# OpenDrift/opendrift

Measured on AMD Instinct MI355X. Metric: particle-steps/sec (RK4, 3D interp), higher is better.
Workload: dtype f64; 1 GPU; C3: OceanDrift 3D, synthetic ROMS-shaped z-level grid 1024x1024x12 (u,v,w,K), RK4 + vertical_mixing(60 s) + vertical_advection; particles_per_gpu=10000000, particles_total=10000000, stage_math=fast, spin_up_steps=200, block_every=0, inputs=resident in HBM, parallelism=particle-sharded x1, field block broadcast once per time level

## Files before the change

include/odrift.h:

```cpp
#ifndef ODRIFT_H
#define ODRIFT_H
#include <stdint.h>

#ifdef __cplusplus
extern "C" {
#endif

typedef struct odr_ctx odr_ctx;
typedef struct odr_particles odr_particles;

typedef enum {
  ODR_OK = 0,
  ODR_ERR_INVALID = -1,
  ODR_ERR_HIP = -2,
  ODR_ERR_CAPACITY = -3,
  ODR_ERR_STATE = -4
} odr_status;

enum {
  ODR_VAR_X_SEA_WATER_VELOCITY = 0,
  ODR_VAR_Y_SEA_WATER_VELOCITY = 1,
  ODR_VAR_X_WIND = 2,
  ODR_VAR_Y_WIND = 3,
  ODR_VAR_UPWARD_SEA_WATER_VELOCITY = 4,
// ... 251 lines not shown
                         double dt_seconds, int rng_mode, const double *u1, const double *u2, const double *diameter_noise,
                         const double *depth_noise, uint64_t step);
int odr_radio_terminal_velocity(odr_ctx *ctx, odr_particles *p, int diameter_slot, int density_slot);
int odr_radio_resuspend(odr_ctx *ctx, odr_particles *p, odr_radio *radio, int specie_slot, int diameter_slot, int rng_mode,
                        const double *diameter_noise, const double *depth_noise, uint64_t step);
int odr_particles_count_status(odr_ctx *ctx, odr_particles *p, int32_t status_code, int64_t *n);
int odr_particles_remap_status(odr_ctx *ctx, odr_particles *p, int32_t from_code, int32_t to_code);
int odr_deactivate(odr_ctx *ctx, odr_particles *p, const uint8_t *mask_host, int32_t status_code);
int odr_deactivate_outside(odr_ctx *ctx, odr_particles *p, double west, double east, double south, double north,
                           int32_t status_code);
int odr_compact(odr_ctx *ctx, odr_particles *p, int64_t *n_active);
int odr_scan_status(odr_ctx *ctx, odr_particles *p, int64_t *n_kept, uint64_t *status_flags);
int odr_scan_status_begin(odr_ctx *ctx, odr_particles *p);
int odr_scan_status_end(odr_ctx *ctx, odr_particles *p, int64_t *n_kept, uint64_t *status_flags);
int odr_ctx_guard_next_vmix(odr_ctx *ctx, int on);
int odr_compact_apply(odr_ctx *ctx, odr_particles *p, int64_t *n_active);
int odr_sort_particles(odr_ctx *ctx, odr_particles *p, int32_t source_id);
int odr_sort_particles_ex(odr_ctx *ctx, odr_particles *p, int32_t source_id, int keep_environment);
int odr_particles_tile_stats(odr_ctx *ctx, odr_particles *p, uint64_t *out4);
int odr_particles_step_layout_stats(odr_ctx *ctx, odr_particles *p, uint64_t *out2);
int odr_particles_step_onlevel_stats(odr_ctx *ctx, odr_particles *p, uint64_t *out1);
int odr_particles_vmix_layout_stats(odr_ctx *ctx, odr_particles *p, uint64_t *out3);
int odr_particles_vmix_kplane_stats(odr_ctx *ctx, odr_particles *p, uint64_t *out2);
int odr_reduce_scalars(odr_ctx *ctx, odr_particles *p, double wind_drift_depth, double *out16);
int odr_ctx_set_step_reduce(odr_ctx *ctx, int on, double wind_drift_depth, int relative_wind);
int odr_reduce_local(odr_ctx *ctx, odr_particles *p, double wind_drift_depth, int relative_wind, double *out16);
int odr_reduce_install(odr_ctx *ctx, odr_particles *p, const double *in16);
int odr_reduce_unpin(odr_ctx *ctx);

int odr_ctx_set_position_class(odr_ctx *ctx, int f32);
int odr_source_set_coordinate_dtype(odr_ctx *ctx, int32_t source_id, int x_is_float32, int y_is_float32);

#define ODR_COMM_ID_BYTES 256
int odr_device_count(int32_t *n);
int odr_comm_unique_id(uint8_t *id );
int odr_comm_init(odr_ctx *ctx, const uint8_t *id, int32_t rank, int32_t nranks);
int odr_comm_info(int32_t *rank, int32_t *nranks, uint64_t *id_hash, int32_t *rccl_version, uint64_t *collectives);
int odr_comm_destroy(void);
int odr_allreduce_scalars(odr_ctx *ctx, double *values, int32_t n, int32_t op);
int odr_comm_allgather_begin(odr_ctx *ctx, const double *row, int32_t n, int32_t from_scan);
int odr_comm_allgather_end(odr_ctx *ctx, double *rows );
int odr_comm_broadcast_bytes(odr_ctx *ctx, void *buf, int64_t nbytes, int32_t root);
int odr_comm_barrier(odr_ctx *ctx);
int odr_block_broadcast(odr_ctx *ctx, int32_t source_id, int32_t slot, double t_epoch, int nvars, const int32_t *var_ids,
                        const void *const *data, const int32_t *var_nz, int ny, int nx, const double *xy8, int32_t root);

// ... 91 lines not shown
```

opendrift_amd/_abi.py:

```python
import ctypes as C
import os

HERE = os.path.dirname(os.path.abspath(__file__))
LIB_PATH = os.environ.get('ODR_LIB') or os.path.join(HERE, 'libodrift_hip.so')

NVAR = 26
VARIABLES = {
    'x_sea_water_velocity': 0, 'y_sea_water_velocity': 1, 'x_wind': 2, 'y_wind': 3,
    'upward_sea_water_velocity': 4, 'ocean_vertical_diffusivity': 5,
    'sea_surface_wave_stokes_drift_x_velocity': 6, 'sea_surface_wave_stokes_drift_y_velocity': 7,
    'land_binary_mask': 8, 'sea_floor_depth_below_sea_level': 9, 'sea_surface_height': 10,
    'horizontal_diffusivity': 11, 'sea_surface_wave_significant_height': 12,
    'sea_surface_wave_period_at_variance_spectral_density_maximum': 13,
    'ocean_mixed_layer_thickness': 14,
    'sea_water_temperature': 15, 'sea_water_salinity': 16,
    'sea_ice_area_fraction': 17, 'sea_ice_x_velocity': 18, 'sea_ice_y_velocity': 19,
    'sea_surface_swell_wave_to_direction': 20,
    'sea_surface_swell_wave_peak_period_from_variance_spectral_density': 21,
    'sea_surface_swell_wave_significant_height': 22, 'sea_surface_wind_wave_to_direction': 23,
    'sea_surface_wind_wave_mean_period': 24, 'sea_surface_wind_wave_significant_height': 25,
}
VARIABLE_NAMES = {v: k for k, v in VARIABLES.items()}
PROJ_LATLONG, PROJ_STERE_EQUIT_SPHERE, PROJ_STERE_POLAR = 0, 1, 2
PROJ_MERC, PROJ_LCC = 4, 5
# ... 151 lines not shown
    'odr_device_count': [_P(C.c_int32)],
    'odr_comm_unique_id': [_P(C.c_uint8)],
    'odr_comm_init': [_vp, _P(C.c_uint8), C.c_int32, C.c_int32],
    'odr_comm_info': [_P(C.c_int32), _P(C.c_int32), _P(C.c_uint64), _P(C.c_int32), _P(C.c_uint64)],
    'odr_comm_destroy': [],
    'odr_allreduce_scalars': [_vp, _dp, C.c_int32, C.c_int32],
    'odr_comm_allgather_begin': [_vp, _dp, C.c_int32, C.c_int32],
    'odr_comm_allgather_end': [_vp, _dp],
    'odr_comm_broadcast_bytes': [_vp, _vp, C.c_int64, C.c_int32],
    'odr_comm_barrier': [_vp],
    'odr_block_broadcast': [_vp, C.c_int32, C.c_int32, C.c_double, C.c_int, _ip, _P(_vp), _ip, C.c_int, C.c_int, _dp, C.c_int32],
    'odr_scan_status': [_vp, _vp, _i64p, _P(C.c_uint64)],
    'odr_scan_status_begin': [_vp, _vp],
    'odr_scan_status_end': [_vp, _vp, _i64p, _P(C.c_uint64)],
    'odr_ctx_guard_next_vmix': [_vp, C.c_int],
    'odr_compact_apply': [_vp, _vp, _i64p],
    'odr_sort_particles': [_vp, _vp, C.c_int32],
    'odr_sort_particles_ex': [_vp, _vp, C.c_int32, C.c_int],
    'odr_particles_tile_stats': [_vp, _vp, _P(C.c_uint64)],
    'odr_particles_step_layout_stats': [_vp, _vp, _P(C.c_uint64)],
    'odr_particles_step_onlevel_stats': [_vp, _vp, _P(C.c_uint64)],
    'odr_particles_vmix_layout_stats': [_vp, _vp, _P(C.c_uint64)],
    'odr_particles_vmix_kplane_stats': [_vp, _vp, _P(C.c_uint64)],
    'odr_reduce_scalars': [_vp, _vp, C.c_double, _dp],
    'odr_ctx_set_step_reduce': [_vp, C.c_int, C.c_double, C.c_int],
    'odr_reduce_local': [_vp, _vp, C.c_double, C.c_int, _dp],
    'odr_reduce_install': [_vp, _vp, _dp],
    'odr_reduce_unpin': [_vp],
    'odr_timer_begin': [_vp],
    'odr_timer_end': [_vp, _fp],
    'odr_sgrid_create': [_vp, C.c_int32, C.c_int32, C.c_int32, _dp, _dp, C.c_double, _dp, _dp, C.c_int32, _P(_vp)],
    'odr_sgrid_destroy': [_vp, _vp],
    'odr_sgrid_download_zrho': [_vp, _vp, _dp],
    'odr_sgrid_zslice': [_vp, _vp, _vp, C.c_int, C.c_int, C.c_int32, _dp, C.c_int32, _P(_vp), _dp],
    'odr_history_create': [_vp, C.c_int64, C.c_int32, C.c_int32, _ip, _P(_vp)],
    'odr_history_destroy': [_vp, _vp],
    'odr_history_set_id_base': [_vp, _vp, C.c_int64],
    'odr_history_record': [_vp, _vp, _vp, C.c_int32, C.c_int, C.c_int],
    'odr_history_flush': [_vp, _vp, C.c_int32, C.c_int32],
    'odr_history_wait': [_vp, _vp],
    'odr_history_host_ptr': [_vp, _vp, C.c_int32, _P(_fp), _P(C.c_int32)],
    'odr_history_reset': [_vp, _vp],
    'odr_history_minmax': [_vp, _vp, C.c_int32, _dp, _dp],
    'odr_density_map': [_vp, C.c_int64, C.c_int32] + [_vp] * 5 + [C.c_int32, C.c_int32, _dp, C.c_int32, _dp, _dp, _dp, _dp],
    'odr_density_last_kernel_ms': [_vp, _fp],
    'odr_density_map_proj': [_vp, C.c_int64, C.c_int32] + [_vp] * 5 + [C.c_int32, _P(ProjDesc), C.c_int32, _dp, C.c_int32, _dp, C.c_int64, _dp, _dp, _dp],
# ... 77 lines not shown
```

opendrift_amd/csrc/odr_host.h:

```cpp
#pragma once
#include <hip/hip_runtime.h>

#include <algorithm>
#include <cmath>
#include <cstdarg>
#include <cstdio>
#include <cstdlib>
#include <cstring>
#include <initializer_list>
#include <string>
#include <vector>

#include "../../include/odrift.h"
#include "odr_kernels.hip.h"

using namespace odr;

#include <chrono>
struct SlowSpan {
  const char *what;
  std::chrono::steady_clock::time_point t0;
  static double limit() { static const double v = getenv("ODR_SLOW_CALLS") ? atof(getenv("ODR_SLOW_CALLS")) : 0.0; return v; }
  explicit SlowSpan(const char *w) : what(w) { if (limit() > 0) t0 = std::chrono::steady_clock::now(); }
  ~SlowSpan() {
// ... 107 lines not shown
  long long aux_snap_cap[9];
  double *dead64[3];
  int *deadi32[2];
  unsigned *bcount;
  unsigned *wcount;
  unsigned long long wcount_epoch;
  long long wcount_n;
  void *scratch;
  size_t scratch_bytes;
  unsigned long long epoch;
  unsigned long long status_epoch, scan_epoch;
  long long scan_kept;
  float env_cval[NVAR];
  long long env_cn[NVAR];
  bool env_cok[NVAR];
  bool external;
  unsigned *wg_tab, *wg_list;
  unsigned long long *wg_total, *wg_stats;
  long long wg_cap, wg_grid, wg_n, wg_list_cap;
  unsigned long long wg_launches;
  unsigned long long step_launches[3];
  unsigned long long vmix_launches[3];
  unsigned long long vmix_kplane[2];
  double *z_keep;
  long long z_keep_n;
  bool z_truncated;
  int wg_sid;
  bool wg_valid;
  unsigned wg_src_gen;
};

static inline unsigned nblk(long long n) { return (unsigned)((n + BLOCK - 1) / BLOCK); }

static inline PView view(const odr_particles *p) {
  PView v;
  v.n = p->n;
  v.lon = p->d64[0]; v.lat = p->d64[1]; v.z = p->d64[2]; v.plon = p->d64[3]; v.plat = p->d64[4];
  v.slon = p->d64[5]; v.slat = p->d64[6];
  v.id = p->i32[0]; v.status = p->i32[1]; v.moving = p->i32[2];
  v.wdf = p->f32[0]; v.cdf = p->f32[1]; v.tv = p->f32[2]; v.age = p->f32[3];
  for (int k = 0; k < NVAR; ++k) v.env[k] = p->env[k];
  for (int k = 0; k < 9; ++k) v.aux[k] = p->aux[k];
  v.ice = p->ice_kind; v.pad = 0;
  v.rank = p->rank_on && p->rank ? p->rank : nullptr;
  return v;
}
// ... 179 lines not shown
```

opendrift_amd/csrc/odr_kernels.hip.h:

```cpp
#pragma once
#include <hip/hip_runtime.h>
#include <rocrand/rocrand_kernel.h>
#include "odr_field.hip.h"

namespace odr {

#ifndef ODR_BLOCK
#define ODR_BLOCK 256
#endif
constexpr int BLOCK = ODR_BLOCK;
#ifndef ODR_POLAR_WAVES
#define ODR_POLAR_WAVES 3
#endif
#ifndef ODR_POLAR_STEP_WAVES
#define ODR_POLAR_STEP_WAVES 2
#endif
#define ODR_STEP_WAVES(PROJ) ((PROJ) == PROJ_LATLONG ? ODR_LATLONG_WAVES : ((PROJ) == PROJ_EXT ? 1 : ODR_POLAR_STEP_WAVES))
#ifndef ODR_LATLONG_WAVES
#define ODR_LATLONG_WAVES 1
#endif
#define ODR_WAVES(PROJ) ((PROJ) == PROJ_LATLONG ? ODR_LATLONG_WAVES : ((PROJ) == PROJ_EXT ? 1 : ODR_POLAR_WAVES))

__device__ __forceinline__ long long pid() {
  const unsigned nb = gridDim.x, b = blockIdx.x, per = nb >> 3, rem = nb & 7u, x = b & 7u, j = b >> 3;
// ... 321 lines not shown
__device__ __forceinline__ unsigned mix_word(const uint4 &q, unsigned k) {
  const unsigned lo = ((q.x & 255u) << 16) | ((q.y & 255u) << 8) | (q.z & 255u);
  return k == 0 ? q.x >> 8 : (k == 1 ? q.y >> 8 : (k == 2 ? q.z >> 8 : (k == 3 ? q.w >> 8 : lo)));
}
__device__ __forceinline__ unsigned mix_draw(const MixKey &K, uint4 &q, int it, bool primed = false) {
  const unsigned b = (unsigned)it / 5u, k = (unsigned)it - 5u * b;
  if (k == 0 && !(primed && it == 0)) q = mix_block(K, b);
  return mix_word(q, k);
}
__device__ __forceinline__ double mix_uniform(const MixKey &K, uint4 &q, int it, bool primed = false) {
  return ((double)mix_draw(K, q, it, primed) + 0.5) * 5.9604644775390625e-08;
}
__device__ __forceinline__ double mix_R_of(unsigned x) {
  return (double)((int)(2u * x + 1u) - (1 << 24)) * 5.9604644775390625e-08;
}
constexpr int AUX_KMEMBER = 8;
struct VMixDesc {
  int sid, nzp, geo_slot;
  unsigned kstride;
  const float *kb, *ka;
  double wgt;
  float Kfb, pad2;
  const unsigned long long *guard;
};

struct VMixRT {
  static constexpr bool STATIC = false;
  __host__ __device__ static constexpr int proj_kind(int k) { return k; }
  __host__ __device__ static constexpr int lon_mode(int m) { return m; }
  __host__ __device__ static constexpr int mod360_x(int m) { return m; }
  __host__ __device__ static constexpr int nzp(int n, int ) { return n; }
  __host__ __device__ static constexpr bool uniform_z(bool u) { return u; }
  __host__ __device__ static constexpr int rng_mode(int m) { return m; }
  __host__ __device__ static constexpr int mix_at_surface(int m) { return m; }
  __host__ __device__ static constexpr int sf_action(int a) { return a; }
  __host__ __device__ static constexpr int vadv(int v) { return v; }
  __host__ __device__ static constexpr int ntimes(int n) { return n; }
  __host__ __device__ static constexpr unsigned kstride(unsigned b, int ) { return b; }
  __device__ static void proj_fwd(const DevProj &p, double lon, double lat, double &x, double &y) { proj_fwd_rt(p, lon, lat, x, y); }
};
struct VMixC3 {
  static constexpr bool STATIC = true;
  __host__ __device__ static constexpr int proj_kind(int) { return PROJ_LATLONG; }
  __host__ __device__ static constexpr int lon_mode(int) { return 1; }
  __host__ __device__ static constexpr int mod360_x(int) { return 0; }
  __host__ __device__ static constexpr int nzp(int, int NL) { return NL; }
  __host__ __device__ static constexpr bool uniform_z(bool) { return false; }
  __host__ __device__ static constexpr int rng_mode(int) { return 0; }
  __host__ __device__ static constexpr int mix_at_surface(int) { return 0; }
  __host__ __device__ static constexpr int sf_action(int) { return 1; }
  __host__ __device__ static constexpr int vadv(int) { return 0; }
  __host__ __device__ static constexpr int ntimes(int) { return 10; }
  __host__ __device__ static constexpr unsigned kstride(unsigned, int NQ) { return 16u * (unsigned)NQ; }
  __device__ static void proj_fwd(const DevProj &, double lon, double lat, double &x, double &y) { x = lon; y = lat; }
};

struct VMixC3Rec : VMixC3 {
  __host__ __device__ static constexpr unsigned kstride(unsigned b, int ) { return b; }
};

template <int NQ, bool TL, class VM, class HOOK>
__device__ __forceinline__ void vmix_col_fill(const DevSource &s, const VMixDesc &D, double lon, double lat, double *Kp,
                                              int tid, HOOK &&hook) {
  const double Kfb = (double)D.Kfb;
  double x, y;
  const int lon_mode = VM::lon_mode(s.lon_mode);
  if (lon_mode == 1) lon = np_mod(lon + 180.0, 360.0) - 180.0;
  else if (lon_mode == 2) lon = np_mod(lon, 360.0);
  VM::proj_fwd(s.proj, lon, lat, x, y);
  const bool cov = x >= s.xmin && x <= s.xmax && y >= s.ymin && y <= s.ymax;
  if (VM::mod360_x(s.mod360_x)) x = np_mod(x, 360.0);
  const DevBlock &bb = s.slot[D.geo_slot];
  const double xi = __dmul_rn(div_cr(x - bb.x0, bb.xspan, bb.ixspan), (double)(bb.nx - 1));
  const double yi = __dmul_rn(div_cr(y - bb.y0, bb.yspan, bb.iyspan), (double)(bb.ny - 1));
  const int ny = bb.ny, nx = bb.nx;
  const Axis ay = axis_fp(yi, ny), ax = axis_fp(xi, nx);
  const double ty = ay.t, tx = ax.t, wy0 = 1 - ty, wx0 = 1 - tx, wgt = D.wgt;
  const unsigned recb = VM::kstride(D.kstride, NQ);
  const unsigned r0 = __umul24((unsigned)ay.i0, (unsigned)nx), r1 = __umul24((unsigned)ay.i1, (unsigned)nx);
  const unsigned o00 = cov ? __umul24(r0 + (unsigned)ax.i0, recb) : 0u, o01 = cov ? __umul24(r0 + (unsigned)ax.i1, recb) : 0u;
  const unsigned o10 = cov ? __umul24(r1 + (unsigned)ax.i0, recb) : 0u, o11 = cov ? __umul24(r1 + (unsigned)ax.i1, recb) : 0u;
  const float *kb = D.kb, *ka = TL ? D.ka : D.kb;
  const double w00 = wy0 * wx0, w01 = wy0 * tx, w10 = ty * wx0, w11 = ty * tx;
#pragma unroll
  for (int q = 0; q < NQ; ++q) {
    if (VM::STATIC && q > 0) __builtin_amdgcn_sched_barrier(0);
    const F4 b00 = ld_off<F4>(kb, o00 + 16u * q), b01 = ld_off<F4>(kb, o01 + 16u * q);
    const F4 b10 = ld_off<F4>(kb, o10 + 16u * q), b11 = ld_off<F4>(kb, o11 + 16u * q);
    F4 a00, a01, a10, a11;
    if (TL) {
      a00 = ld_off<F4>(ka, o00 + 16u * q); a01 = ld_off<F4>(ka, o01 + 16u * q);
      a10 = ld_off<F4>(ka, o10 + 16u * q); a11 = ld_off<F4>(ka, o11 + 16u * q);
    }
    if (VM::STATIC && q > 0) __builtin_amdgcn_sched_barrier(0);
    if (q == 0) hook();
    double v[4];
    v[0] = (double)bilw(b00.x, b01.x, b10.x, b11.x, w00, w01, w10, w11);
    v[1] = (double)bilw(b00.y, b01.y, b10.y, b11.y, w00, w01, w10, w11);
    v[2] = (double)bilw(b00.z, b01.z, b10.z, b11.z, w00, w01, w10, w11);
    v[3] = (double)bilw(b00.w, b01.w, b10.w, b11.w, w00, w01, w10, w11);
    if (TL) {
      double w[4];
      w[0] = (double)bilw(a00.x, a01.x, a10.x, a11.x, w00, w01, w10, w11);
      w[1] = (double)bilw(a00.y, a01.y, a10.y, a11.y, w00, w01, w10, w11);
      w[2] = (double)bilw(a00.z, a01.z, a10.z, a11.z, w00, w01, w10, w11);
      w[3] = (double)bilw(a00.w, a01.w, a10.w, a11.w, w00, w01, w10, w11);
#pragma unroll
      for (int j = 0; j < 4; ++j) v[j] = __dadd_rn(__dmul_rn(v[j], 1 - wgt), __dmul_rn(w[j], wgt));
// ... 2 lines not shown
    for (int j = 0; j < 4; ++j) Kp[(4 * q + j) * BLOCK + tid] = (cov && isfinite(v[j])) ? v[j] : Kfb;
  }
}

struct VMixArgs {
  double dt, dt_mix_cfg;
  int mix_at_surface, rng_mode, sfl, pad;
  const double *huni;
  unsigned long long seed, step;
};
struct MixRng { MixKey key; uint4 q; bool primed; };
template <class VM = VMixRT>
__device__ __forceinline__ MixRng mix_rng_begin(const VMixArgs &A, int id) {
  MixRng R;
  R.key = mix_key(A.seed, A.step, id);
  R.q = make_uint4(0u, 0u, 0u, 0u);
  R.primed = false;
  if (VM::rng_mode(A.rng_mode) == 0) {
    R.q = mix_block(R.key, 0u);
    R.primed = true;
  }
  return R;
}
template <int NQ, class VM = VMixRT>
__device__ __forceinline__ double vmix_col_walk(const DevSource &s, int nzp, const double *Kp, const double *gsh, int tid,
                                                const VMixArgs &A, long long i, long long n, int id, double z, int &moving,
                                                float Zmin, float tv, int &sf_flags, const MixRng *pre) {
  constexpr int NL = 4 * NQ;
  static_assert(!VM::STATIC || NL >= 3, "a static configuration has the three-level window inside the profile");
  const double dt = A.dt;
  const int mix_at_surface = VM::mix_at_surface(A.mix_at_surface), rng_mode = VM::rng_mode(A.rng_mode), sfl = A.sfl;
  double zm[NL - 1];
#pragma unroll
  for (int k = 0; k < NL - 1; ++k) zm[k] = k < nzp - 1 ? s.zmid[k] : __builtin_inf();
  const bool uniform_z = VM::uniform_z(s.vg_uniform != 0);
  const double gd0 = s.vg_d[0], gi0 = s.vg_id[0], gd1 = s.vg_d[1], gi1 = s.vg_id[1], gd2 = s.vg_d[2], gi2 = s.vg_id[2];
  const double sgn = dt > 0 ? 1.0 : (dt < 0 ? -1.0 : 0.0);
  const double dt_mix = A.dt_mix_cfg * sgn;
  const int ntimes = VM::ntimes(abs((int)(dt / dt_mix)));
  const double r = 1.0 / 3, ir = 1.0 / r;
  double wstep = __dmul_rn(__dmul_rn((double)tv, dt_mix), (double)moving);
  const MixKey st = mix_key(A.seed, A.step, id);
  uint4 u4 = make_uint4(0u, 0u, 0u, 0u);
  bool primed = false;
  if (pre) { u4 = pre->q; primed = pre->primed; }
  auto level_terms = [&](auto edges, int zl, double &dk_dt, double &sg) {
    constexpr int E = decltype(edges)::value;
    const double Kz = Kp[zl * BLOCK + tid];
    double gK;
    if ((E & 1) && zl == 0) gK = div_cr(Kp[BLOCK + tid] - Kz, gd0, gi0);
    else if ((E & 2) && zl == nzp - 1) gK = div_cr(Kz - Kp[(nzp - 2) * BLOCK + tid], gd1, gi1);
    else if (uniform_z) gK = div_cr(Kp[(zl + 1) * BLOCK + tid] - Kp[(zl - 1) * BLOCK + tid], gd2, gi2);
    else
      gK = __dadd_rn(__dadd_rn(__dmul_rn(gsh[zl], Kp[(zl - 1) * BLOCK + tid]), __dmul_rn(gsh[NL + zl], Kz)),
                     __dmul_rn(gsh[2 * NL + zl], Kp[(zl + 1) * BLOCK + tid]));
    double dK = -gK;
    if (fabs(dK) < 1e-10) dK = 0;
    dk_dt = __dmul_rn(dK, dt_mix);
    sg = sqrt(div_cr(__dmul_rn(__dmul_rn(Kz, fabs(dt_mix)), 2.0), r, ir));
  };
  using AnyLevel = std::integral_constant<int, 3>;
  int lv0;
  {
    const double d0 = -z;
    int zs = 0;
#pragma unroll
    for (int k = 0; k < NL - 1; ++k) zs += ((k & 1) ? d0 >= zm[k] : d0 > zm[k]) ? 1 : 0;
    lv0 = zs < 1 ? 1 : (zs > nzp - 2 ? nzp - 2 : zs);
    if (nzp < 3) lv0 = 1;
  }
  double c_dk[3], c_sg[3];
#pragma unroll
  for (int q = 0; q < 3; ++q) {
    const int zl = lv0 - 1 + q;
    c_dk[q] = 0; c_sg[q] = 0;
    if constexpr (VM::STATIC) {
      if (q == 0) level_terms(std::integral_constant<int, 1>(), zl, c_dk[q], c_sg[q]);
      else if (q == 1) level_terms(std::integral_constant<int, 0>(), zl, c_dk[q], c_sg[q]);
      else level_terms(std::integral_constant<int, 2>(), zl, c_dk[q], c_sg[q]);
    } else if (zl >= 0 && zl < nzp) level_terms(AnyLevel(), zl, c_dk[q], c_sg[q]);
  }
  double wb[4];
#pragma unroll
  for (int j = 0; j < 4; ++j) {
    const int k = lv0 - 2 + j;
    double b = k < 0 ? -1.0 : __builtin_inf();
    if (k >= 0 && k < nzp - 1) {
      b = gsh[3 * NL + k];
      if ((k & 1) && b > 0) b = __longlong_as_double(__double_as_longlong(b) - 1);
    }
    wb[j] = b;
  }
  for (int it0 = 0; it0 < ntimes; it0 += 5) {
  if (rng_mode == 0 && !(primed && it0 == 0)) u4 = mix_block(st, (unsigned)it0 / 5u);
#pragma unroll
  for (int k5 = 0; k5 < 5; ++k5) {
    const int it = it0 + k5;
    if (it >= ntimes) break;
    const bool surface = z == 0;
    const double d = -z;
    int q = (d > wb[1] ? 1 : 0) + (d > wb[2] ? 1 : 0);
    int zi = lv0 - 1 + q;
    if (!(d > wb[0]) || d > wb[3]) {
      zi = 0;
#pragma unroll
      for (int k = 0; k < NL - 1; ++k) zi += ((k & 1) ? d >= zm[k] : d > zm[k]) ? 1 : 0;
      q = zi - lv0 + 1;
    }
    double dKdt = q == 0 ? c_dk[0] : (q == 1 ? c_dk[1] : c_dk[2]);
    double sig = q == 0 ? c_sg[0] : (q == 1 ? c_sg[1] : c_sg[2]);
    if (q < 0 || q > 2) level_terms(AnyLevel(), zi, dKdt, sig);
    double R;
    if (rng_mode == 1) R = __dsub_rn(__dmul_rn(2.0, A.huni[(size_t)it * n + i]), 1.0);
    else R = mix_R_of(mix_word(u4, (unsigned)k5));
    z = __dsub_rn(z, __dmul_rn((double)moving, __dsub_rn(dKdt, __dmul_rn(R, sig))));
    if (z >= 0) z = -z;
    if (z < (double)Zmin && moving == 1) z = __dsub_rn((double)__fmul_rn(2.f, Zmin), z);
    z = __dadd_rn(z, wstep);
    if (!mix_at_surface && surface) z = 0.0;
    if (z > 0) z = 0.0;
    if (z < (double)Zmin) {
      const int act = VM::sf_action(sfl & 255);
      if (act == 3) sf_flags |= 2;
      else if (act) {
        z = (double)Zmin;
        if (act == 2) { sf_flags |= 1; moving = 0; wstep = 0.0; }
        else if (act == 4) { sf_flags |= 4; moving = 0; wstep = 0.0; }
        else if (act == 5 && (sf_flags & 8)) { sf_flags |= 4; moving = 0; wstep = 0.0; }
      }
    }
  }
  }
  return z;
}
// ... 1047 lines not shown
  if (vadv >= 0 && (vadv ? z <= 0 : z < 0)) {
    double zz = __dadd_rn(z, __dmul_rn(__dmul_rn((double)moving, (double)p.env[VAR_W][i]), dt));
    z = zz < 0 ? zz : 0.0;
  }
  if (OIL) {
    p.tv[i] = (float)oil.W;
    p.aux[OIL_DIAMETER][i] = oil.d;
  }
  p.z[i] = z;
}

#ifndef ODR_VMIX_WAVES
#define ODR_VMIX_WAVES 6
#endif
struct VMixState { double slon, slat, z0; int moving, id; float dep, ssh, tv; };
__device__ __forceinline__ VMixState vmix_load_state(const PView &p, long long i) {
  VMixState S;
  S.slon = p.slon[i]; S.slat = p.slat[i]; S.z0 = p.z[i];
  S.moving = p.moving[i]; S.id = p.id[i];
  S.dep = p.env[VAR_DEPTH][i]; S.ssh = p.env[VAR_SSH][i]; S.tv = p.tv[i];
  return S;
}
template <int NQ, bool TL, class VM>
__device__ __forceinline__ void vmix_col_particle(const DevSource &s, const PView &p, const VMixDesc &D, const VMixArgs &A,
                                                  int vadv, long long i, double *Kp, const double *gsh, int tid, const VMixState &S) {
  const int nzp = VM::nzp(D.nzp, 4 * NQ), sfl = A.sfl;
  const double dt = A.dt;
  const double slon = S.slon, slat = S.slat, z0 = S.z0;
  int moving = S.moving;
  const float dep0 = S.dep, ssh0 = S.ssh, tv0 = S.tv;
  const int id0 = S.id;
  MixRng R0;
  R0.key = mix_key(A.seed, A.step, id0); R0.q = make_uint4(0u, 0u, 0u, 0u); R0.primed = false;
  vmix_col_fill<NQ, TL, VM>(s, D, slon, slat, Kp, tid, [&]() { R0 = mix_rng_begin<VM>(A, id0); });
  int sf_flags = VM::sf_action(sfl & 255) == 5 ? sf_species_flag(p, sfl, i) : 0;
  const float Zmin = __fmul_rn(-1.f, __fadd_rn(dep0, ssh0));
  double z = vmix_col_walk<NQ, VM>(s, nzp, Kp, gsh, tid, A, i, p.n, id0, z0, moving, Zmin, tv0, sf_flags, &R0);
  if (sf_flags & 1) {
    if (p.status[i] == 0) p.status[i] = sfl >> 8;
    p.moving[i] = 0;
  }
  if (sf_flags & 4) p.moving[i] = 0;
  if (sf_flags & 2) { p.lon[i] = p.plon[i]; p.lat[i] = p.plat[i]; }
  vadv = VM::vadv(vadv);
  if (vadv >= 0 && (vadv ? z <= 0 : z < 0)) {
    const float w0 = p.env[VAR_W][i];
    double zz = __dadd_rn(z, __dmul_rn(__dmul_rn((double)moving, (double)w0), dt));
    z = zz < 0 ? zz : 0.0;
  }
  p.z[i] = z;
}
template <int NQ, bool TL, class VM = VMixRT>
__global__ __launch_bounds__(BLOCK, ODR_VMIX_WAVES) void k_vmix_col(const DevWorld *__restrict__ W, PView p, VMixDesc D,
                                                    double dt, double dt_mix_cfg, int mix_at_surface,
                                                    int rng_mode, const double *__restrict__ huni,
                                                    unsigned long long seed, unsigned long long step,
                                                    int vadv, int sfl) {
  constexpr int NL = 4 * NQ;
  extern __shared__ __attribute__((aligned(16))) char smem[];
  const int tid = threadIdx.x;
  const DevSource &s = W->src[D.sid];
  const int nzp = VM::nzp(D.nzp, NL);
  double *Kp = (double *)smem;
  double *gsh = Kp + (size_t)NL * BLOCK;
  if (D.guard && *D.guard == 0ull) return;
  const long long i = pid();
  const bool valid = i < p.n;
  const VMixState S = vmix_load_state(p, valid ? i : 0);
  if (tid < nzp) {
    gsh[tid] = s.vg_a[tid]; gsh[NL + tid] = s.vg_b[tid]; gsh[2 * NL + tid] = s.vg_c[tid];
    gsh[3 * NL + tid] = s.zmid[tid];
  }
  __syncthreads();
  if (!valid) return;
  VMixArgs A;
  A.dt = dt; A.dt_mix_cfg = dt_mix_cfg; A.mix_at_surface = mix_at_surface; A.rng_mode = rng_mode; A.sfl = sfl; A.pad = 0;
  A.huni = huni; A.seed = seed; A.step = step;
  vmix_col_particle<NQ, TL, VM>(s, p, D, A, vadv, i, Kp, gsh, tid, S);
}

#ifndef ODR_VWIN_WAVES
#define ODR_VWIN_WAVES 5
#endif
template <bool TL>
__device__ __forceinline__ double vmix_layer(float b00, float b01, float b10, float b11, float a00, float a01, float a10, float a11,
                                             double w00, double w01, double w10, double w11, double wgt, bool cov, double Kfb) {
  double v = (double)bilw(b00, b01, b10, b11, w00, w01, w10, w11);
  if (TL) {
    const double w = (double)bilw(a00, a01, a10, a11, w00, w01, w10, w11);
    v = __dadd_rn(__dmul_rn(v, 1 - wgt), __dmul_rn(w, wgt));
  }
  return (cov && isfinite(v)) ? v : Kfb;
}
struct VMixGrad { double gd0, gi0, gd1, gi1, gd2, gi2, dt_mix; bool uniform_z; };
__device__ __forceinline__ void vmix_terms(const VMixGrad &G, const double *gsh, int nzp, int zl, double Kl, double Kz, double Kh,
                                           double &dk_dt, double &sg) {
  const double r = 1.0 / 3, ir = 1.0 / r;
  double gK;
  if (zl == 0) gK = div_cr(Kh - Kz, G.gd0, G.gi0);
  else if (zl == nzp - 1) gK = div_cr(Kz - Kl, G.gd1, G.gi1);
  else if (G.uniform_z) gK = div_cr(Kh - Kl, G.gd2, G.gi2);
// ... 1448 lines not shown
```

opendrift_amd/csrc/odr_mix.hip:

```cpp
#define ODR_TU_MIX 1
#include "odr_host.h"

template <class VM>
static bool vmix_layout_matches(const DevSource &s, const VMixDesc &D, int nq, double dt, double dt_mix, int mix_at_surface,
                                int rng_mode, int sfl, int vadv) {
  const bool uz = s.vg_uniform != 0;
  const int ntimes = abs((int)(dt / (dt_mix * (dt > 0 ? 1.0 : (dt < 0 ? -1.0 : 0.0)))));
  return VM::proj_kind(s.proj.kind) == s.proj.kind && VM::lon_mode(s.lon_mode) == s.lon_mode &&
         VM::mod360_x(s.mod360_x) == s.mod360_x && VM::nzp(D.nzp, 4 * nq) == D.nzp && VM::uniform_z(uz) == uz &&
         VM::rng_mode(rng_mode) == rng_mode && VM::mix_at_surface(mix_at_surface) == mix_at_surface &&
         VM::sf_action(sfl & 255) == (sfl & 255) && VM::vadv(vadv) == vadv && VM::ntimes(ntimes) == ntimes &&
         VM::kstride(D.kstride, nq) == D.kstride;
}

int odr_vmix(odr_ctx *c, odr_particles *p, double t, double dt, double dt_mix, int mix_at_surface, int rng_mode,
             const double *huni, uint64_t step) {
  const bool guarded = c->guard_next_vmix != 0;
  c->guard_next_vmix = 0;
  const bool oil = c->oil_owner == p;
  const bool f32prof = p->profiles_f32;
  const int cut = c->vmix_levels;
  VMixDesc D;
  bool kplanes = !getenv("ODR_NO_KPLANE");
  const bool fast = !oil && !f32prof && cut <= 0 && !getenv("ODR_NO_FAST_PATH") && build_vmix_desc(c, t, D, kplanes);
// ... 34 lines not shown
  unsigned long long st = (unsigned long long)step;
  if (vadv >= 0 && !p->env[VAR_W]) return fail(ODR_ERR_STATE, "upward_sea_water_velocity has not been sampled");
  struct F32ProfileClass {
    odr_ctx *c;
    bool on;
    ~F32ProfileClass() { if (on) { c->hw.f32pos &= ~2; c->dirty = true; } }
  } f32bit{c, false};
  if (f32prof) { c->hw.f32pos |= 2; c->dirty = true; f32bit.on = true; if ((rc = flush_world(c))) return rc; }
  if (cut > 0) {
    REQUIRE(cut >= 2 && cut <= 255, "odr_vmix_set_profile_levels: 2 .. 255 levels");
    if (cut < nzp) nzp = cut;
  }
  const int sfl_cut = c->seafloor | ((cut > 0 ? nzp : 0) << 16);
  if (fast) {
    if (guarded) { D.guard = c->counter + 4; c->guarded_vmix = p; c->guarded_vadv = vadv; }
    const int nq = (nzp + 3) / 4;
    const bool tl = D.ka != nullptr;
    const char *wenv = getenv("ODR_VMIX_WINDOW");
    const bool win = nzp >= 3 && nzp <= BLOCK && (wenv ? atoi(wenv) != 0 : nzp > 12);
    const bool spec = !win && (nq == 2 || nq == 3) &&
                      vmix_layout_matches<VMixC3Rec>(c->hw.src[D.sid], D, nq, dt, dt_mix, mix_at_surface, rng_mode, c->seafloor, vadv) &&
                      !getenv("ODR_NO_VMIX_SPEC");
    const bool specp = spec && vmix_layout_matches<VMixC3>(c->hw.src[D.sid], D, nq, dt, dt_mix, mix_at_surface, rng_mode, c->seafloor, vadv);
    p->vmix_launches[win ? 2 : spec ? 1 : 0]++;
    p->vmix_kplane[kplanes ? 0 : 1]++;
#define VMIX_COL(NQ, VM)                                                                                          \
  do {                                                                                                            \
    size_t l2 = sizeof(double) * ((size_t)(4 * NQ) * BLOCK + 4 * (size_t)(4 * NQ));                               \
    if (tl) hipLaunchKernelGGL((k_vmix_col<NQ, true, VM>), g, b, l2, c->stream, c->dw, v, D, dt, dt_mix,          \
                               mix_at_surface, rng_mode, du, c->seed, st, vadv, c->seafloor);                                  \
    else hipLaunchKernelGGL((k_vmix_col<NQ, false, VM>), g, b, l2, c->stream, c->dw, v, D, dt, dt_mix,            \
                            mix_at_surface, rng_mode, du, c->seed, st, vadv, c->seafloor);                                     \
  } while (0)
    if (win) {
      const size_t lw = (sizeof(double) + sizeof(unsigned)) * 4 * BLOCK + sizeof(double) * 4 * (size_t)nzp;
      if (tl) hipLaunchKernelGGL((k_vmix_win<true>), g, b, lw, c->stream, c->dw, v, D, dt, dt_mix, mix_at_surface, rng_mode, du,
                                 c->seed, st, vadv, c->seafloor);
      else hipLaunchKernelGGL((k_vmix_win<false>), g, b, lw, c->stream, c->dw, v, D, dt, dt_mix, mix_at_surface, rng_mode, du,
                              c->seed, st, vadv, c->seafloor);
    }
    else if (specp && nq == 2) VMIX_COL(2, VMixC3);
    else if (specp) VMIX_COL(3, VMixC3);
    else if (spec && nq == 2) VMIX_COL(2, VMixC3Rec);
    else if (spec) VMIX_COL(3, VMixC3Rec);
    else if (nq <= 1) VMIX_COL(1, VMixRT);
    else if (nq == 2) VMIX_COL(2, VMixRT);
    else if (nq == 3) VMIX_COL(3, VMixRT);
    else if (nq == 4) VMIX_COL(4, VMixRT);
    else if (nq <= 6) VMIX_COL(6, VMixRT);
    else if (nq <= 8) VMIX_COL(8, VMixRT);
    else if (nq <= 12) VMIX_COL(12, VMixRT);
    else VMIX_COL(16, VMixRT);
#undef VMIX_COL
  } else if (oil) {
    if (nzp <= 16) hipLaunchKernelGGL((k_vmix<16, true>), g, b, lds, c->stream, c->dw, v, t, dt, dt_mix, mix_at_surface, rng_mode, du, c->seed, st, vadv, sfl_cut, c->oil);
    else if (nzp <= 32) hipLaunchKernelGGL((k_vmix<32, true>), g, b, lds, c->stream, c->dw, v, t, dt, dt_mix, mix_at_surface, rng_mode, du, c->seed, st, vadv, sfl_cut, c->oil);
    else hipLaunchKernelGGL((k_vmix<1, true>), g, b, lds, c->stream, c->dw, v, t, dt, dt_mix, mix_at_surface, rng_mode, du, c->seed, st, vadv, sfl_cut, c->oil);
  } else if (nzp <= 16) hipLaunchKernelGGL(k_vmix<16>, g, b, lds, c->stream, c->dw, v, t, dt, dt_mix, mix_at_surface, rng_mode, du, c->seed, st, vadv, sfl_cut);
  else if (nzp <= 32) hipLaunchKernelGGL(k_vmix<32>, g, b, lds, c->stream, c->dw, v, t, dt, dt_mix, mix_at_surface, rng_mode, du, c->seed, st, vadv, sfl_cut);
  else hipLaunchKernelGGL(k_vmix<1>, g, b, lds, c->stream, c->dw, v, t, dt, dt_mix, mix_at_surface, rng_mode, du, c->seed, st, vadv, sfl_cut);
  if (!fast) p->vmix_launches[2]++;
  HIPCHK(hipGetLastError());
  return 0;
}

int odr_particles_vmix_layout_stats(odr_ctx *c, odr_particles *p, uint64_t *out3) {
  REQUIRE(c && p && out3, "NULL argument");
  for (int k = 0; k < 3; ++k) out3[k] = p->vmix_launches[k];
  return 0;
}

int odr_particles_vmix_kplane_stats(odr_ctx *c, odr_particles *p, uint64_t *out2) {
  REQUIRE(c && p && out2, "NULL argument");
  out2[0] = p->vmix_kplane[0]; out2[1] = p->vmix_kplane[1];
  return 0;
}

int odr_vmix_set_profile_levels(odr_ctx *c, int32_t n) {
  REQUIRE(n == 0 || (n >= 2 && n <= 255), "bad level count %d", n);
  c->vmix_levels = n;
  return 0;
}

int odr_vmix_wind_profile(odr_ctx *c, odr_particles *p, int model, double background_diffusivity, double dt,
                          double dt_mix, int mix_at_surface, int rng_mode, const double *huni, uint64_t step) {
  c->guard_next_vmix = 0;
  p->status_epoch++;
  p->epoch++;
  REQUIRE(model == ODR_DIFFUSIVITY_LARGE1994 || model == ODR_DIFFUSIVITY_SUNDBY1983, "Unknown diffusivity model: %d", model);
  REQUIRE(dt_mix > 0 && dt != 0, "bad time steps");
  if (!p->env[VAR_DEPTH]) return fail(ODR_ERR_STATE, "sea_floor_depth_below_sea_level has not been sampled");
  int rc;
  if ((rc = seafloor_species_slot_ok(c, p))) return rc;
  for (int v : {VAR_SSH, VAR_XWIND, VAR_YWIND, VAR_MLD})
    if ((rc = ensure_env(c, p, v))) return rc;
  if ((rc = flush_world(c))) return rc;
  if (p->n == 0) return 0;
// ... 162 lines not shown
```

opendrift_amd/csrc/odrift.hip:

```cpp
#define ODR_TU_MISC 1
#include "odr_host.h"
#include "odr_mesh.h"

static thread_local std::string g_err;
int odr_i_fail(int code, const char *fmt, ...) {
  char buf[512];
  va_list ap;
  va_start(ap, fmt);
  vsnprintf(buf, sizeof buf, fmt, ap);
  va_end(ap);
  g_err = buf;
  return code;
}

const char *odr_last_error(void) { return g_err.c_str(); }
#define ODR_STR2(x) #x
#define ODR_STR(x) ODR_STR2(x)
const char *odr_version(void) { return "odrift-hip 0.2 (gfx950; mixing stream Philox4x32-" ODR_STR(ODR_MIX_ROUNDS) ")"; }

int odr_ctx_create(int device, uint64_t seed, odr_ctx **out) {
  REQUIRE(out, "out is NULL");
  HIPCHK(hipSetDevice(device));
  odr_ctx *c = new odr_ctx();
  c->device = device;
// ... 79 lines not shown
  return 0;
}
int odr_timer_end(odr_ctx *c, float *ms) {
  HIPCHK(hipEventRecord(c->ev1, c->stream));
  HIPCHK(hipEventSynchronize(c->ev1));
  HIPCHK(hipEventElapsedTime(ms, c->ev0, c->ev1));
  return 0;
}

int odr_particles_create(odr_ctx *c, int64_t capacity, odr_particles **out) {
  REQUIRE(capacity > 0 && out, "capacity must be positive");
  HIPCHK(hipSetDevice(c->device));
  odr_particles *p = new odr_particles();
  memset(p, 0, sizeof(*p));
  p->cap = capacity;
  p->dead_cap = capacity;
  p->scan_kept = -1;
  for (int k = 0; k < 7; ++k) HIPCHK(hipMalloc((void **)&p->d64[k], sizeof(double) * (size_t)capacity));
  for (int k = 0; k < 3; ++k) HIPCHK(hipMalloc((void **)&p->i32[k], sizeof(int) * (size_t)capacity));
  for (int k = 0; k < 4; ++k) HIPCHK(hipMalloc((void **)&p->f32[k], sizeof(float) * (size_t)capacity));
  HIPCHK(hipMalloc((void **)&p->bcount, sizeof(unsigned) * (size_t)(nblk(capacity) + 1)));
  HIPCHK(hipMalloc((void **)&p->wcount, sizeof(unsigned) * (size_t)(nblk(capacity) + 1) * (BLOCK / 64)));
  p->wcount_epoch = ~0ull;
  *out = p;
  return 0;
}

int odr_particles_destroy(odr_ctx *c, odr_particles *p) {
  if (c->red_owner == p) c->red_owner = nullptr;
  if (c->noise_owner == p) c->noise_owner = nullptr;
  if (c->guarded_vmix == p) c->guarded_vmix = nullptr;
  if (!p) return 0;
  (void)hipStreamSynchronize(c->stream);
  auto fr = [](void *q) { if (q) (void)hipFree(q); };
  for (int k = 0; k < 7; ++k) { fr(p->d64[k]); fr(p->alt64[k]); }
  for (int k = 0; k < 3; ++k) { fr(p->i32[k]); fr(p->alti32[k]); fr(p->dead64[k]); }
  for (int k = 0; k < 4; ++k) { fr(p->f32[k]); fr(p->altf32[k]); }
  for (int k = 0; k < 2; ++k) fr(p->deadi32[k]);
  for (int k = 0; k < NVAR; ++k) { fr(p->env[k]); fr(p->altenv[k]); }
  for (int k = 0; k < 9; ++k) { fr(p->aux[k]); fr(p->altaux[k]); fr(p->aux_snap[k]); }
  fr(p->bcount);
  fr(p->wcount);
  fr(p->scratch);
  fr(p->rank); fr(p->rank_words); fr(p->rank_before); fr(p->rank_bsum);
  fr(p->wg_tab); fr(p->wg_total); fr(p->wg_list); fr(p->z_keep);
  delete p;
  return 0;
}

template <class T>
static int put(odr_ctx *c, T *dst, const T *src, long long n, T dflt) {
  if (src) {
    H2D(dst, src, sizeof(T) * (size_t)n);
  } else {
    std::vector<T> tmp((size_t)n, dflt);
    H2D(dst, tmp.data(), sizeof(T) * (size_t)n);
    HIPCHK(hipStreamSynchronize(c->stream));
  }
  return 0;
}

int odr_particles_append(odr_ctx *c, odr_particles *p, int64_t n, const double *lon, const double *lat,
                         const double *z, const int32_t *id, const int32_t *moving, const float *wdf,
                         const float *cdf, const float *tv) {
  p->status_epoch++;
// ... 2410 lines not shown
```

opendrift_amd/device.py:

```python
import ctypes as C
import os

import numpy as np

from . import _abi
from ._abi import VARIABLES, check

_dp, _fp, _ip = C.POINTER(C.c_double), C.POINTER(C.c_float), C.POINTER(C.c_int32)


def _vid(v, aliases=None):
    if isinstance(v, (int, np.integer)):
        return v
    if v in VARIABLES:
        return VARIABLES[v]
    if aliases and v in aliases:
        return aliases[v]
    raise KeyError(v)


def _d(a, n=None):
    if a is None:
        return None, None
    a = np.ascontiguousarray(np.broadcast_to(np.asarray(a, dtype=np.float64), (n,)) if n is not None
# ... 1152 lines not shown
        import ctypes as C
        out = (C.c_uint64 * 2)()
        check(self.lib.odr_particles_step_layout_stats(self.ctx.h, self.h, out))
        return dict(runtime=int(out[0]), static=int(out[1]))

    def step_onlevel_stats(self):
        import ctypes as C
        out = (C.c_uint64 * 1)()
        check(self.lib.odr_particles_step_onlevel_stats(self.ctx.h, self.h, out))
        return int(out[0])

    def vmix_layout_stats(self):
        import ctypes as C
        out = (C.c_uint64 * 3)()
        check(self.lib.odr_particles_vmix_layout_stats(self.ctx.h, self.h, out))
        return dict(runtime=int(out[0]), static=int(out[1]), other=int(out[2]))

    def vmix_kplane_stats(self):
        import ctypes as C
        out = (C.c_uint64 * 2)()
        check(self.lib.odr_particles_vmix_kplane_stats(self.ctx.h, self.h, out))
        return dict(planes=int(out[0]), records=int(out[1]))

    def reduce_global(self, combine, wind_drift_depth=0.1, relative_wind=False):
        raw = np.empty(16)
        check(self.lib.odr_reduce_local(self.ctx.h, self.h, float(wind_drift_depth), int(relative_wind), raw.ctypes.data_as(_dp)))
        g = np.ascontiguousarray(combine(raw), dtype=np.float64)
        check(self.lib.odr_reduce_install(self.ctx.h, self.h, g.ctypes.data_as(_dp)))
        return g

    def reduce_local(self, wind_drift_depth=0.1, relative_wind=False):
        raw = np.empty(16)
        check(self.lib.odr_reduce_local(self.ctx.h, self.h, float(wind_drift_depth), int(relative_wind), raw.ctypes.data_as(_dp)))
        return raw

    def reduce_install(self, combined16):
        g = np.ascontiguousarray(combined16, dtype=np.float64)
        check(self.lib.odr_reduce_install(self.ctx.h, self.h, g.ctypes.data_as(_dp)))

    @staticmethod
    def reduction_dict(raw):
        keys = ['n_active', 'lon_min', 'lon_max', 'lat_min', 'lat_max', 'z_min', 'z_max', 'D_max',
                'stokes_sum_max', 'wind_speed_max', 'wdf_surface_max', 'n_surface', 'hs_max', 'tp_max']
        d = dict(zip(keys, raw))
        for k in ('lon_min', 'lat_min', 'z_min'):
            d[k] = -d[k]
# ... 319 lines not shown
```

Measured before the change: 11.37 billion particle-steps/s.

## Fill only a two-quad vertical window of K column in vmix, redo on escape

For the static C3 vertical-mixing path with three quads (12 levels), each particle now loads only the two 4-level quads of the diffusivity column around its starting level instead of all three. If the random walk leaves the loaded window, the particle's state is reloaded and the full three-quad kernel path is rerun for it. This cuts global/LDS loads of K per particle, at the cost of extra register pressure, a ballot, and divergent full recomputation for escaping particles. A counter and stats API report how many particles were redone.

```diff
diff --git a/include/odrift.h b/include/odrift.h
--- a/include/odrift.h
+++ b/include/odrift.h
@@ -297,6 +297,7 @@
 int odr_particles_step_onlevel_stats(odr_ctx *ctx, odr_particles *p, uint64_t *out1);
 int odr_particles_vmix_layout_stats(odr_ctx *ctx, odr_particles *p, uint64_t *out3);
 int odr_particles_vmix_kplane_stats(odr_ctx *ctx, odr_particles *p, uint64_t *out2);
+int odr_particles_vmix_window_stats(odr_ctx *ctx, odr_particles *p, uint64_t *out3);
 int odr_reduce_scalars(odr_ctx *ctx, odr_particles *p, double wind_drift_depth, double *out16);
 int odr_ctx_set_step_reduce(odr_ctx *ctx, int on, double wind_drift_depth, int relative_wind);
 int odr_reduce_local(odr_ctx *ctx, odr_particles *p, double wind_drift_depth, int relative_wind, double *out16);
diff --git a/opendrift_amd/_abi.py b/opendrift_amd/_abi.py
--- a/opendrift_amd/_abi.py
+++ b/opendrift_amd/_abi.py
@@ -197,6 +197,7 @@
     'odr_particles_step_onlevel_stats': [_vp, _vp, _P(C.c_uint64)],
     'odr_particles_vmix_layout_stats': [_vp, _vp, _P(C.c_uint64)],
     'odr_particles_vmix_kplane_stats': [_vp, _vp, _P(C.c_uint64)],
+    'odr_particles_vmix_window_stats': [_vp, _vp, _P(C.c_uint64)],
     'odr_reduce_scalars': [_vp, _vp, C.c_double, _dp],
     'odr_ctx_set_step_reduce': [_vp, C.c_int, C.c_double, C.c_int],
     'odr_reduce_local': [_vp, _vp, C.c_double, C.c_int, _dp],
diff --git a/opendrift_amd/csrc/odr_host.h b/opendrift_amd/csrc/odr_host.h
--- a/opendrift_amd/csrc/odr_host.h
+++ b/opendrift_amd/csrc/odr_host.h
@@ -153,6 +153,8 @@
   unsigned long long step_launches[3];
   unsigned long long vmix_launches[3];
   unsigned long long vmix_kplane[2];
+  unsigned long long vmix_window[2];
+  unsigned long long *vmix_redone;
   double *z_keep;
   long long z_keep_n;
   bool z_truncated;
diff --git a/opendrift_amd/csrc/odr_kernels.hip.h b/opendrift_amd/csrc/odr_kernels.hip.h
--- a/opendrift_amd/csrc/odr_kernels.hip.h
+++ b/opendrift_amd/csrc/odr_kernels.hip.h
@@ -367,10 +367,12 @@
   double wgt;
   float Kfb, pad2;
   const unsigned long long *guard;
+  unsigned long long *redone;
 };
 
 struct VMixRT {
   static constexpr bool STATIC = false;
+  static constexpr bool WINDOW = false;
   __host__ __device__ static constexpr int proj_kind(int k) { return k; }
   __host__ __device__ static constexpr int lon_mode(int m) { return m; }
   __host__ __device__ static constexpr int mod360_x(int m) { return m; }
@@ -386,6 +388,7 @@
 };
 struct VMixC3 {
   static constexpr bool STATIC = true;
+  static constexpr bool WINDOW = false;
   __host__ __device__ static constexpr int proj_kind(int) { return PROJ_LATLONG; }
   __host__ __device__ static constexpr int lon_mode(int) { return 1; }
   __host__ __device__ static constexpr int mod360_x(int) { return 0; }
@@ -403,10 +406,21 @@
 struct VMixC3Rec : VMixC3 {
   __host__ __device__ static constexpr unsigned kstride(unsigned b, int ) { return b; }
 };
+struct VMixWin { int lv0, q0; bool escaped; };
+struct VMixC3W : VMixC3 {
+  static constexpr bool WINDOW = true;
+  using Full = VMixC3;
+};
+struct VMixC3RecW : VMixC3Rec {
+  static constexpr bool WINDOW = true;
+  using Full = VMixC3Rec;
+};
 
 template <int NQ, bool TL, class VM, class HOOK>
 __device__ __forceinline__ void vmix_col_fill(const DevSource &s, const VMixDesc &D, double lon, double lat, double *Kp,
-                                              int tid, HOOK &&hook) {
+                                              int tid, int q0, HOOK &&hook) {
+  static_assert(!VM::WINDOW || NQ >= 2, "a two-quad configuration needs two quads");
+  constexpr int NF = VM::WINDOW ? 2 : NQ;
   const double Kfb = (double)D.Kfb;
   double x, y;
   const int lon_mode = VM::lon_mode(s.lon_mode);
@@ -423,12 +437,17 @@
   const double ty = ay.t, tx = ax.t, wy0 = 1 - ty, wx0 = 1 - tx, wgt = D.wgt;
   const unsigned recb = VM::kstride(D.kstride, NQ);
   const unsigned r0 = __umul24((unsigned)ay.i0, (unsigned)nx), r1 = __umul24((unsigned)ay.i1, (unsigned)nx);
-  const unsigned o00 = cov ? __umul24(r0 + (unsigned)ax.i0, recb) : 0u, o01 = cov ? __umul24(r0 + (unsigned)ax.i1, recb) : 0u;
-  const unsigned o10 = cov ? __umul24(r1 + (unsigned)ax.i0, recb) : 0u, o11 = cov ? __umul24(r1 + (unsigned)ax.i1, recb) : 0u;
+  unsigned o00 = cov ? __umul24(r0 + (unsigned)ax.i0, recb) : 0u, o01 = cov ? __umul24(r0 + (unsigned)ax.i1, recb) : 0u;
+  unsigned o10 = cov ? __umul24(r1 + (unsigned)ax.i0, recb) : 0u, o11 = cov ? __umul24(r1 + (unsigned)ax.i1, recb) : 0u;
+  if constexpr (VM::WINDOW) {
+    const unsigned qb = 16u * (unsigned)q0;
+    o00 += qb; o01 += qb; o10 += qb; o11 += qb;
+    Kp += 4 * q0 * BLOCK;
+  }
   const float *kb = D.kb, *ka = TL ? D.ka : D.kb;
   const double w00 = wy0 * wx0, w01 = wy0 * tx, w10 = ty * wx0, w11 = ty * tx;
 #pragma unroll
-  for (int q = 0; q < NQ; ++q) {
+  for (int q = 0; q < NF; ++q) {
     if (VM::STATIC && q > 0) __builtin_amdgcn_sched_barrier(0);
     const F4 b00 = ld_off<F4>(kb, o00 + 16u * q), b01 = ld_off<F4>(kb, o01 + 16u * q);
     const F4 b10 = ld_off<F4>(kb, o10 + 16u * q), b11 = ld_off<F4>(kb, o11 + 16u * q);
@@ -477,17 +496,31 @@
   }
   return R;
 }
+template <int NL>
+__device__ __forceinline__ void vmix_level_bounds(const DevSource &s, int nzp, double (&zm)[NL - 1]) {
+#pragma unroll
+  for (int k = 0; k < NL - 1; ++k) zm[k] = k < nzp - 1 ? s.zmid[k] : __builtin_inf();
+}
+template <int NL>
+__device__ __forceinline__ int vmix_start_level(const double (&zm)[NL - 1], int nzp, double z) {
+  const double d0 = -z;
+  int zs = 0;
+#pragma unroll
+  for (int k = 0; k < NL - 1; ++k) zs += ((k & 1) ? d0 >= zm[k] : d0 > zm[k]) ? 1 : 0;
+  int lv0 = zs < 1 ? 1 : (zs > nzp - 2 ? nzp - 2 : zs);
+  if (nzp < 3) lv0 = 1;
+  return lv0;
+}
 template <int NQ, class VM = VMixRT>
 __device__ __forceinline__ double vmix_col_walk(const DevSource &s, int nzp, const double *Kp, const double *gsh, int tid,
                                                 const VMixArgs &A, long long i, long long n, int id, double z, int &moving,
-                                                float Zmin, float tv, int &sf_flags, const MixRng *pre) {
+                                                float Zmin, float tv, int &sf_flags, const MixRng *pre, VMixWin *win = nullptr) {
   constexpr int NL = 4 * NQ;
   static_assert(!VM::STATIC || NL >= 3, "a static configuration has the three-level window inside the profile");
   const double dt = A.dt;
   const int mix_at_surface = VM::mix_at_surface(A.mix_at_surface), rng_mode = VM::rng_mode(A.rng_mode), sfl = A.sfl;
   double zm[NL - 1];
-#pragma unroll
-  for (int k = 0; k < NL - 1; ++k) zm[k] = k < nzp - 1 ? s.zmid[k] : __builtin_inf();
+  vmix_level_bounds<NL>(s, nzp, zm);
   const bool uniform_z = VM::uniform_z(s.vg_uniform != 0);
   const double gd0 = s.vg_d[0], gi0 = s.vg_id[0], gd1 = s.vg_d[1], gi1 = s.vg_id[1], gd2 = s.vg_d[2], gi2 = s.vg_id[2];
   const double sgn = dt > 0 ? 1.0 : (dt < 0 ? -1.0 : 0.0);
@@ -516,14 +549,8 @@
   };
   using AnyLevel = std::integral_constant<int, 3>;
   int lv0;
-  {
-    const double d0 = -z;
-    int zs = 0;
-#pragma unroll
-    for (int k = 0; k < NL - 1; ++k) zs += ((k & 1) ? d0 >= zm[k] : d0 > zm[k]) ? 1 : 0;
-    lv0 = zs < 1 ? 1 : (zs > nzp - 2 ? nzp - 2 : zs);
-    if (nzp < 3) lv0 = 1;
-  }
+  if constexpr (VM::WINDOW) lv0 = win->lv0;
+  else lv0 = vmix_start_level<NL>(zm, nzp, z);
   double c_dk[3], c_sg[3];
 #pragma unroll
   for (int q = 0; q < 3; ++q) {
@@ -564,7 +591,13 @@
     }
     double dKdt = q == 0 ? c_dk[0] : (q == 1 ? c_dk[1] : c_dk[2]);
     double sig = q == 0 ? c_sg[0] : (q == 1 ? c_sg[1] : c_sg[2]);
-    if (q < 0 || q > 2) level_terms(AnyLevel(), zi, dKdt, sig);
+    if (q < 0 || q > 2) {
+      if constexpr (VM::WINDOW) {
+        const int lo = zi > 0 ? zi - 1 : 0, hi = zi < nzp - 1 ? zi + 1 : nzp - 1;
+        if (lo < 4 * win->q0 || hi > 4 * win->q0 + 7) win->escaped = true;
+      }
+      level_terms(AnyLevel(), zi, dKdt, sig);
+    }
     double R;
     if (rng_mode == 1) R = __dsub_rn(__dmul_rn(2.0, A.huni[(size_t)it * n + i]), 1.0);
     else R = mix_R_of(mix_word(u4, (unsigned)k5));
@@ -1658,7 +1691,7 @@
   return S;
 }
 template <int NQ, bool TL, class VM>
-__device__ __forceinline__ void vmix_col_particle(const DevSource &s, const PView &p, const VMixDesc &D, const VMixArgs &A,
+__device__ __forceinline__ bool vmix_col_particle(const DevSource &s, const PView &p, const VMixDesc &D, const VMixArgs &A,
                                                   int vadv, long long i, double *Kp, const double *gsh, int tid, const VMixState &S) {
   const int nzp = VM::nzp(D.nzp, 4 * NQ), sfl = A.sfl;
   const double dt = A.dt;
@@ -1668,10 +1701,20 @@
   const int id0 = S.id;
   MixRng R0;
   R0.key = mix_key(A.seed, A.step, id0); R0.q = make_uint4(0u, 0u, 0u, 0u); R0.primed = false;
-  vmix_col_fill<NQ, TL, VM>(s, D, slon, slat, Kp, tid, [&]() { R0 = mix_rng_begin<VM>(A, id0); });
+  VMixWin win = {0, 0, false};
+  if constexpr (VM::WINDOW) {
+    double zm[4 * NQ - 1];
+    vmix_level_bounds<4 * NQ>(s, nzp, zm);
+    win.lv0 = vmix_start_level<4 * NQ>(zm, nzp, z0);
+    const int qa = (win.lv0 > 2 ? win.lv0 - 2 : 0) >> 2;
+    win.q0 = qa < NQ - 2 ? qa : NQ - 2;
+  }
+  vmix_col_fill<NQ, TL, VM>(s, D, slon, slat, Kp, tid, win.q0, [&]() { R0 = mix_rng_begin<VM>(A, id0); });
   int sf_flags = VM::sf_action(sfl & 255) == 5 ? sf_species_flag(p, sfl, i) : 0;
   const float Zmin = __fmul_rn(-1.f, __fadd_rn(dep0, ssh0));
-  double z = vmix_col_walk<NQ, VM>(s, nzp, Kp, gsh, tid, A, i, p.n, id0, z0, moving, Zmin, tv0, sf_flags, &R0);
+  double z = vmix_col_walk<NQ, VM>(s, nzp, Kp, gsh, tid, A, i, p.n, id0, z0, moving, Zmin, tv0, sf_flags, &R0,
+                                   VM::WINDOW ? &win : nullptr);
+  if (VM::WINDOW && win.escaped) return true;
   if (sf_flags & 1) {
     if (p.status[i] == 0) p.status[i] = sfl >> 8;
     p.moving[i] = 0;
@@ -1685,6 +1728,7 @@
     z = zz < 0 ? zz : 0.0;
   }
   p.z[i] = z;
+  return false;
 }
 template <int NQ, bool TL, class VM = VMixRT>
 __global__ __launch_bounds__(BLOCK, ODR_VMIX_WAVES) void k_vmix_col(const DevWorld *__restrict__ W, PView p, VMixDesc D,
@@ -1712,7 +1756,17 @@
   VMixArgs A;
   A.dt = dt; A.dt_mix_cfg = dt_mix_cfg; A.mix_at_surface = mix_at_surface; A.rng_mode = rng_mode; A.sfl = sfl; A.pad = 0;
   A.huni = huni; A.seed = seed; A.step = step;
-  vmix_col_particle<NQ, TL, VM>(s, p, D, A, vadv, i, Kp, gsh, tid, S);
+  const bool escaped = vmix_col_particle<NQ, TL, VM>(s, p, D, A, vadv, i, Kp, gsh, tid, S);
+  if constexpr (VM::WINDOW) {
+    const unsigned long long esc = __ballot(escaped);
+    if (esc != 0ull) {
+      if (escaped) {
+        const VMixState S2 = vmix_load_state(p, i);
+        vmix_col_particle<NQ, TL, typename VM::Full>(s, p, D, A, vadv, i, Kp, gsh, tid, S2);
+        if (D.redone && (tid & 63) == __ffsll((long long)esc) - 1) atomicAdd(D.redone, (unsigned long long)__popcll(esc));
+      }
+    }
+  }
 }
 
 #ifndef ODR_VWIN_WAVES
diff --git a/opendrift_amd/csrc/odr_mix.hip b/opendrift_amd/csrc/odr_mix.hip
--- a/opendrift_amd/csrc/odr_mix.hip
+++ b/opendrift_amd/csrc/odr_mix.hip
@@ -80,8 +80,11 @@
                       vmix_layout_matches<VMixC3Rec>(c->hw.src[D.sid], D, nq, dt, dt_mix, mix_at_surface, rng_mode, c->seafloor, vadv) &&
                       !getenv("ODR_NO_VMIX_SPEC");
     const bool specp = spec && vmix_layout_matches<VMixC3>(c->hw.src[D.sid], D, nq, dt, dt_mix, mix_at_surface, rng_mode, c->seafloor, vadv);
+    const bool quadwin = spec && nq == 3 && !getenv("ODR_NO_VMIX_WINDOW");
     p->vmix_launches[win ? 2 : spec ? 1 : 0]++;
     p->vmix_kplane[kplanes ? 0 : 1]++;
+    if (spec && nq == 3) p->vmix_window[quadwin ? 0 : 1]++;
+    D.redone = quadwin ? p->vmix_redone : nullptr;
 #define VMIX_COL(NQ, VM)                                                                                          \
   do {                                                                                                            \
     size_t l2 = sizeof(double) * ((size_t)(4 * NQ) * BLOCK + 4 * (size_t)(4 * NQ));                               \
@@ -98,8 +101,10 @@
                               c->seed, st, vadv, c->seafloor);
     }
     else if (specp && nq == 2) VMIX_COL(2, VMixC3);
+    else if (specp && quadwin) VMIX_COL(3, VMixC3W);
     else if (specp) VMIX_COL(3, VMixC3);
     else if (spec && nq == 2) VMIX_COL(2, VMixC3Rec);
+    else if (spec && quadwin) VMIX_COL(3, VMixC3RecW);
     else if (spec) VMIX_COL(3, VMixC3Rec);
     else if (nq <= 1) VMIX_COL(1, VMixRT);
     else if (nq == 2) VMIX_COL(2, VMixRT);
@@ -131,6 +136,15 @@
 int odr_particles_vmix_kplane_stats(odr_ctx *c, odr_particles *p, uint64_t *out2) {
   REQUIRE(c && p && out2, "NULL argument");
   out2[0] = p->vmix_kplane[0]; out2[1] = p->vmix_kplane[1];
+  return 0;
+}
+
+int odr_particles_vmix_window_stats(odr_ctx *c, odr_particles *p, uint64_t *out3) {
+  REQUIRE(c && p && out3, "NULL argument");
+  unsigned long long redone = 0;
+  D2H(&redone, p->vmix_redone, sizeof redone);
+  HIPCHK(hipStreamSynchronize(c->stream));
+  out3[0] = p->vmix_window[0]; out3[1] = p->vmix_window[1]; out3[2] = redone;
   return 0;
 }
 
diff --git a/opendrift_amd/csrc/odrift.hip b/opendrift_amd/csrc/odrift.hip
--- a/opendrift_amd/csrc/odrift.hip
+++ b/opendrift_amd/csrc/odrift.hip
@@ -125,6 +125,8 @@
   HIPCHK(hipMalloc((void **)&p->bcount, sizeof(unsigned) * (size_t)(nblk(capacity) + 1)));
   HIPCHK(hipMalloc((void **)&p->wcount, sizeof(unsigned) * (size_t)(nblk(capacity) + 1) * (BLOCK / 64)));
   p->wcount_epoch = ~0ull;
+  HIPCHK(hipMalloc((void **)&p->vmix_redone, sizeof(unsigned long long)));
+  HIPCHK(hipMemset(p->vmix_redone, 0, sizeof(unsigned long long)));
   *out = p;
   return 0;
 }
@@ -144,6 +146,7 @@
   for (int k = 0; k < 9; ++k) { fr(p->aux[k]); fr(p->altaux[k]); fr(p->aux_snap[k]); }
   fr(p->bcount);
   fr(p->wcount);
+  fr(p->vmix_redone);
   fr(p->scratch);
   fr(p->rank); fr(p->rank_words); fr(p->rank_before); fr(p->rank_bsum);
   fr(p->wg_tab); fr(p->wg_total); fr(p->wg_list); fr(p->z_keep);
diff --git a/opendrift_amd/device.py b/opendrift_amd/device.py
--- a/opendrift_amd/device.py
+++ b/opendrift_amd/device.py
@@ -1198,6 +1198,12 @@
         check(self.lib.odr_particles_vmix_kplane_stats(self.ctx.h, self.h, out))
         return dict(planes=int(out[0]), records=int(out[1]))
 
+    def vmix_window_stats(self):
+        import ctypes as C
+        out = (C.c_uint64 * 3)()
+        check(self.lib.odr_particles_vmix_window_stats(self.ctx.h, self.h, out))
+        return dict(windowed=int(out[0]), full=int(out[1]), redone=int(out[2]))
+
     def reduce_global(self, combine, wind_drift_depth=0.1, relative_wind=False):
         raw = np.empty(16)
         check(self.lib.odr_reduce_local(self.ctx.h, self.h, float(wind_drift_depth), int(relative_wind), raw.ctypes.data_as(_dp)))
```

New measurement: 11.74 billion particle-steps/s, median of 6. 1.03x the previous value.
